# Lexmata/llama-gguf

Measured on AMD Instinct MI355X. Metric: decode tokens/sec Llama-3-8B Q4_K_M, 1 GPU; % of HBM roofline, higher is better.
Workload: dtype f32 (x as 4xint8 limbs on the matrix cores, exact int32 accumulation)

## Files before the change

### llama-gguf_amd/csrc/attention.hip

```cpp
#include <cstdlib>

#include "attn_split.h"
#include "tq_fwht.h"
#include "xq.h"
#include "prefill.h"
#include "timeline.h"

LGH_TL_DEFINE(attn)

namespace lgh {

template <int D, int G, int NW, bool PF = false, bool DIRECT = false, bool MULTI = false>
__global__ void __launch_bounds__(NW * 64) attn_partial_kernel(const float* __restrict__ q, const float* __restrict__ kc,
                                                           const float* __restrict__ vc, uint32_t max_seq, float scale,
                                                           const int* pos_ptr, int kv_len_fixed, uint32_t n_splits,
                                                           float* __restrict__ part_ml, float* __restrict__ part_acc,
                                                           const int* __restrict__ slot = nullptr, uint64_t slot_stride = 0) {
  constexpr int LPR = D / 4;
  constexpr int RPW = 64 / LPR;
  __shared__ float s_ml[NW * G * 2];
  __shared__ __attribute__((aligned(16))) float s_acc[NW * G * D];
  LGH_TL_BEGIN(attn, lgh::TL_ATTN, n_splits);

  const uint32_t kvh = blockIdx.x / n_splits, sp = blockIdx.x % n_splits;
// ... 43 lines not shown
#pragma unroll
    for (int j = 0; j < kAhead; j++)
      if (base + j * stride < kv_len) step(base + j * stride, kk[j], vv[j]);
  }

  attn_merge_rows<G, LPR>(m, l, acc);
  attn_stash<G, 4, LPR>(s_ml, s_acc, wave, sub, li, m, l, acc);
  __syncthreads();
  const size_t pbase = ((size_t)kvh * n_splits + sp) * G;
  for (uint32_t e = threadIdx.x; e < (uint32_t)(G * D); e += NW * 64) {
    const uint32_t g = e / D, dim = e % D;
    float mn, lsum, a;
    attn_merge_waves<NW, G, D>(s_ml, s_acc, g, dim, mn, lsum, a);
    if (DIRECT) {
      const float o = a * (1.0f / lsum);
      part_acc[(pbase + g) * D + dim] = o;
      if (part_ml) xq_store_chunk(reinterpret_cast<uint8_t*>(part_ml), (uint32_t)((pbase + g) * D + dim) >> 4, o);
    } else if (PF) {
      const _Float16 o = (_Float16)(a * (1.0f / lsum));
      *reinterpret_cast<_Float16*>(reinterpret_cast<uint8_t*>(part_acc) + xh_offset(blockIdx.y, (uint32_t)(pbase + g) * D + dim)) = o;
    } else {
      attn_store_partial<D>(part_ml, part_acc, pbase + g, dim, mn, lsum, a);
    }
  }
  LGH_TL_END();
}

__device__ __forceinline__ f32x4 unpack_i8x4(uint32_t w, float scale) {
  f32x4 r;
  r.x = (float)(int)(int8_t)(w & 0xFFu) * scale;
  r.y = (float)(int)(int8_t)((w >> 8) & 0xFFu) * scale;
  r.z = (float)(int)(int8_t)((w >> 16) & 0xFFu) * scale;
  r.w = (float)(int)(int8_t)(w >> 24) * scale;
  return r;
}

__device__ __forceinline__ float i8_row_scale(float amax) { return amax > 1e-10f ? amax / 127.0f : 1.0f; }
__device__ __forceinline__ uint32_t i8_quantize(float v, float scale) {
  float r = roundf(v / scale);
  r = r < -128.0f ? -128.0f : (r > 127.0f ? 127.0f : r);
  return (uint32_t)(int)r & 0xFFu;
}

template <int LPR>
__device__ __forceinline__ uint32_t quantize_row_i8(f32x4 x, float& scale) {
  float amax = fmaxf(fmaxf(fabsf(x.x), fabsf(x.y)), fmaxf(fabsf(x.z), fabsf(x.w)));
// ... 262 lines not shown
    constexpr int D = decltype(d)::value, G = decltype(gg)::value;
    return long_ctx ? attn_go<D, G, 8>(a) : attn_go<D, G, 4>(a);
  });
}

hipError_t attn_launch(const float* q, const float* kcache, const float* vcache, uint32_t n_heads, uint32_t n_kv,
                       uint32_t head_dim, uint32_t max_seq, float scale, const int* pos, int kv_len_fixed,
                       uint32_t n_splits, float* part_ml, float* part_acc, hipStream_t st) {
  if (n_kv == 0 || n_heads % n_kv) return hipErrorInvalidValue;
  return attn_split_dispatch(head_dim, n_heads / n_kv,
                             AttnArgs{q, kcache, vcache, n_kv, max_seq, scale, pos, kv_len_fixed, n_splits, part_ml, part_acc, st, 0, nullptr, 0});
}

hipError_t attn_direct_launch(const float* q, const float* kcache, const float* vcache, uint32_t n_heads, uint32_t n_kv, uint32_t head_dim,
                              uint32_t max_seq, float scale, const int* pos, float* out, uint8_t* xq_out, hipStream_t st) {
  if (n_kv == 0 || n_heads % n_kv || !pos) return hipErrorInvalidValue;
  return attn_dispatch(head_dim, n_heads / n_kv, [&](auto d, auto gg) {
    hipLaunchKernelGGL((attn_partial_kernel<decltype(d)::value, decltype(gg)::value, 16, false, true>), dim3(n_kv), dim3(1024), 0, st, q, kcache, vcache,
                       max_seq, scale, pos, 0, 1u, reinterpret_cast<float*>(xq_out), out);
    return hipGetLastError();
  });
}

struct PfTqEpi { const float* signs; float inv_scale, inv_d; };

template <int D, int NW, bool TQ>
__global__ void __launch_bounds__(NW * 64) attn_pf_mfma_kernel(const float* __restrict__ q, const float* __restrict__ kc, const float* __restrict__ vc,
                                                               uint32_t n_heads, uint32_t g_per_kv, uint32_t max_seq, float scale, uint32_t pos0,
                                                               uint32_t m_tokens, uint8_t* __restrict__ xh_out, const PfTqEpi tq) {
  constexpr int DJ = D / 4;
  constexpr int DQ = D / 16;
  constexpr int DP = D + 4;
  extern __shared__ __attribute__((aligned(16))) float pf_lds[];
  float (*s_o)[16][DP] = reinterpret_cast<float (*)[16][DP]>(pf_lds);
  float (*s_m)[16] = reinterpret_cast<float (*)[16]>(pf_lds + NW * 16 * DP);
  float (*s_l)[16] = s_m + NW;
  const uint32_t head = blockIdx.x, tt = blockIdx.y, kvh = head / g_per_kv;
  const uint32_t lane = threadIdx.x & 63, wave = threadIdx.x >> 6, n = lane & 15, c = lane >> 4;
  const uint32_t tok = tt * 16 + n, tokc = tok < m_tokens ? tok : m_tokens - 1;
  const uint32_t kv_last = pos0 + m_tokens - 1;
  const uint32_t n_tiles = (pos0 + tt * 16 + 16 + 15) / 16;
  float qf[DJ];
  {
    const float* qp = q + ((size_t)tokc * n_heads + head) * D + c * DJ;
#pragma unroll
    for (int j = 0; j < DJ; j += 4) {
// ... 249 lines not shown
```

### llama-gguf_amd/csrc/common.h

```cpp
#pragma once

#include <hip/hip_runtime.h>
#include <stdint.h>
#include <stddef.h>
#include <vector>

#include "../../include/llama_gguf_hip.h"

namespace lgh {

typedef uint32_t u32x4 __attribute__((ext_vector_type(4)));
typedef uint32_t u32x2 __attribute__((ext_vector_type(2)));
typedef float f32x4 __attribute__((ext_vector_type(4)));

constexpr int kWave = 64;
constexpr int kNumCU = 256;

__host__ __device__ inline uint32_t blk_elems(int t) {
  switch (t) {
    case LGH_TYPE_F32: case LGH_TYPE_F16: case LGH_TYPE_BF16: return 1;
    case LGH_TYPE_Q4_0: case LGH_TYPE_Q4_1: case LGH_TYPE_Q5_0: case LGH_TYPE_Q5_1: case LGH_TYPE_Q8_0:
    case LGH_TYPE_Q8_1: return 32;
    case LGH_TYPE_Q2_K: case LGH_TYPE_Q3_K: case LGH_TYPE_Q4_K: case LGH_TYPE_Q5_K: case LGH_TYPE_Q6_K:
    case LGH_TYPE_Q8_K: return 256;
// ... 159 lines not shown
                             uint32_t n_splits, float* part_ml, float* part_acc, hipStream_t st);
hipError_t attn_combine_multi_launch(const float* part_ml, const float* part_acc, uint32_t n_heads, uint32_t n_kv, uint32_t head_dim,
                                     uint32_t n_splits, uint32_t n_seq, float* out, uint8_t* xq_out, hipStream_t st);
hipError_t ewise_launch(int op, const float* a, const float* b, float s, float* out, uint64_t n, hipStream_t st);
hipError_t softmax_rows_launch(const float* x, float* out, uint32_t rows, uint32_t last_dim, hipStream_t st);
hipError_t matmul_f32_launch(const float* a, const float* b, float* c, uint32_t m, uint32_t k, uint32_t n, hipStream_t st);
hipError_t silu_mul_launch(const float* gate, const float* up, float* out, uint32_t n, hipStream_t st);
hipError_t argmax_launch(const float* logits, uint32_t n, float* part_val, int* part_idx, int* state, int* out_token,
                         hipStream_t st);
hipError_t argmax_merge_launch(const float* part_val, const int* part_idx, uint32_t nparts, int* state, int* out_token, hipStream_t st);
hipError_t advance_launch(int* state, hipStream_t st);
hipError_t copy_words_launch(void* dst, const void* src, uint32_t n_words, hipStream_t st);
hipError_t moe_group_launch(const int* sel, uint32_t n_seq, uint32_t top_k, uint32_t n_experts, int* cnt, int* idx, uint32_t idx_stride, hipStream_t st);
hipError_t moe_combine_launch(const float* tmp, const float* moe_w, uint32_t top_k, float* hidden, uint32_t H, uint32_t n_seq, const float* nw,
                              uint8_t* xq, uint32_t xq_stride, float* ssq, uint32_t ssq_stride, hipStream_t st);
hipError_t moe_router_launch(const float* x, const float* norm_w, float eps, const float* w, uint32_t hidden,
                             uint32_t n_experts, uint32_t top_k, int* sel, float* sel_w, hipStream_t st, uint32_t n_tokens = 1);

hipError_t attn_launch(const float* q, const float* kcache, const float* vcache, uint32_t n_heads, uint32_t n_kv,
                       uint32_t head_dim, uint32_t max_seq, float scale, const int* pos, int kv_len_fixed,
                       uint32_t n_splits, float* part_ml, float* part_acc, hipStream_t st);
hipError_t attn_direct_launch(const float* q, const float* kcache, const float* vcache, uint32_t n_heads, uint32_t n_kv, uint32_t head_dim,
                              uint32_t max_seq, float scale, const int* pos, float* out, uint8_t* xq_out, hipStream_t st);
bool attn_shape_has_fast_kernel(uint32_t head_dim, uint32_t group);
hipError_t kv_roundtrip_launch(int fmt, const float* x, uint32_t n, uint8_t* bytes, float* scale_out, float* back, hipStream_t st);
hipError_t attn_q8_launch(int fmt, const float* q, int8_t* k8, int8_t* v8, float* kscale, float* vscale, const float* k_new, const float* v_new,
                          uint32_t n_heads, uint32_t n_kv, uint32_t head_dim, uint32_t max_seq, float scale, const int* pos, uint32_t n_splits,
                          float* part_ml, float* part_acc, hipStream_t st);
hipError_t attn_q8_multi_launch(int fmt, const float* q, int8_t* k8, int8_t* v8, float* kscale, float* vscale, const float* k_new, const float* v_new,
                                uint32_t x_stride, uint32_t n_heads, uint32_t n_kv, uint32_t head_dim, uint32_t max_seq, float scale, const int* pos,
                                const int* slot, uint32_t n_seq, uint32_t n_splits, float* part_ml, float* part_acc, hipStream_t st);
hipError_t attn_tq_launch(int bits, const float* q, uint8_t* kq, uint8_t* vq, const float* k_new, const float* v_new, const float* signs,
                          uint32_t n_heads, uint32_t n_kv, uint32_t head_dim, uint32_t max_seq, float scale, const int* pos, uint32_t n_splits,
                          float* part_ml, float* part_acc, hipStream_t st, const float* qjl_s = nullptr, uint32_t* kx = nullptr);
hipError_t attn_tq_combine_launch(int bits, const float* part_ml, const float* part_acc, const float* signs, uint32_t n_heads, uint32_t n_kv,
                                  uint32_t head_dim, uint32_t n_splits, float* out, uint8_t* xq_out, hipStream_t st, uint32_t n_seq = 0,
                                  uint32_t xq_stride = 0);
hipError_t attn_tq_multi_launch(int bits, const float* q, uint8_t* kq, uint8_t* vq, const float* k_new, const float* v_new, const float* signs,
                                uint32_t n_heads, uint32_t n_kv, uint32_t head_dim, uint32_t max_seq, float scale, const int* pos, const int* slot,
                                uint64_t code_stride, uint64_t x_stride, uint32_t kv_stride, uint32_t n_seq, uint32_t n_splits, float* part_ml,
                                float* part_acc, hipStream_t st, const float* qjl_s = nullptr, uint32_t* kx = nullptr);
hipError_t tq_compress_launch(int bits, const float* x, uint32_t dim, const float* signs, uint8_t* out, hipStream_t st, const float* qjl_s = nullptr,
                              uint32_t* qjl_out = nullptr);
uint32_t tq_row_bytes_host(int bits, uint32_t d);
hipError_t tq_pf_rows_launch(int bits, float* kscr, float* vscr, uint8_t* kq, uint8_t* vq, float* q, const float* signs, uint32_t n_heads,
                             uint32_t n_kv, uint32_t head_dim, uint32_t max_seq, uint32_t pos0, uint32_t m_store, uint32_t m_q, uint32_t n_expand,
// ... 25 lines not shown
```

### llama-gguf_amd/csrc/device_utils.h

```cpp
#pragma once

#include "common.h"

namespace lgh {

__device__ __forceinline__ u32x4 ldg_nt128(const void* p) {
  return __builtin_nontemporal_load(reinterpret_cast<const u32x4*>(p));
}
__device__ __forceinline__ u32x2 ldg_nt64(const void* p) {
  return __builtin_nontemporal_load(reinterpret_cast<const u32x2*>(p));
}
__device__ __forceinline__ uint32_t ldg_nt32(const void* p) {
  return __builtin_nontemporal_load(reinterpret_cast<const uint32_t*>(p));
}
__device__ __forceinline__ uint16_t ldg_nt16(const void* p) {
  return __builtin_nontemporal_load(reinterpret_cast<const uint16_t*>(p));
}

__device__ __forceinline__ float h2f(uint32_t bits16) {
  _Float16 h;
  uint16_t b = (uint16_t)bits16;
  __builtin_memcpy(&h, &b, 2);
  return (float)h;
}
// ... 34 lines not shown
}

__device__ __forceinline__ float wave_sum(float v) {
#pragma unroll
  for (int off = 32; off >= 1; off >>= 1) v += __shfl_xor(v, off, 64);
  return v;
}

template <int CTRL, int ROW_MASK = 0xF>
__device__ __forceinline__ float dpp_f(float v) {
  return __builtin_bit_cast(float, __builtin_amdgcn_update_dpp(0, __builtin_bit_cast(int, v), CTRL, ROW_MASK, 0xF, false));
}

__device__ __forceinline__ float wave_sum_to_lane63(float v) {
  v += dpp_f<0xB1>(v);
  v += dpp_f<0x4E>(v);
  v += dpp_f<0x141>(v);
  v += dpp_f<0x140>(v);
  v += dpp_f<0x142, 0xA>(v);
  v += dpp_f<0x143, 0xC>(v);
  return v;
}

__device__ __forceinline__ float wave_max(float v) {
#pragma unroll
  for (int off = 32; off >= 1; off >>= 1) v = fmaxf(v, __shfl_xor(v, off, 64));
  return v;
}

__device__ __forceinline__ void amax_merge(float& bv, int& bi, float v, int i) {
  if (v > bv || (v == bv && i > bi)) { bv = v; bi = i; }
}

__device__ __forceinline__ void amax_block_reduce(float& bv, int& bi, float* sv, int* si) {
#pragma unroll
  for (int off = 32; off >= 1; off >>= 1) {
    float ov = __shfl_xor(bv, off, 64);
    int oi = __shfl_xor(bi, off, 64);
    amax_merge(bv, bi, ov, oi);
  }
  const uint32_t tid = threadIdx.x;
  if ((tid & 63) == 0) { sv[tid >> 6] = bv; si[tid >> 6] = bi; }
  __syncthreads();
  if (tid == 0) {
    for (uint32_t w = 1; w < (blockDim.x >> 6); w++) amax_merge(bv, bi, sv[w], si[w]);
  }
// ... 4 lines not shown
```

### llama-gguf_amd/csrc/engine.h

```cpp
#pragma once

#include <functional>
#include <string>
#include <vector>

#include "common.h"
#include "kv_cache.h"
#include "sample.h"

namespace lgh {

struct LayerW {
  bool owned = false;
  DevWeight wq, wk, wv, wo, gate, up, down;
  DevWeight gate_exps, up_exps, down_exps;
  float* attn_norm = nullptr;
  float* ffn_norm = nullptr;
  float* router = nullptr;
  float* bq = nullptr; float* bk = nullptr; float* bv = nullptr; float* bo = nullptr;
  KvCache kv;
  bool moe() const { return router != nullptr; }
};

enum TokenMode { MODE_PREFILL = 0, MODE_FORWARD = 1, MODE_GREEDY = 2, MODE_SAMPLE = 3, MODE_COUNT = 4 };

struct XqBuf { const float* f32 = nullptr; uint8_t* xq = nullptr; float* ssq = nullptr; uint32_t k = 0; bool fresh = false; const float* tag = nullptr; };

struct PfScratch {
  bool ready = false;
  uint8_t *xh_h = nullptr, *xh_attn = nullptr, *xh_act = nullptr;
  float *hidden = nullptr, *q = nullptr, *part = nullptr, *ssq = nullptr;
  size_t part_bytes = 0;
  int* tokens = nullptr;
  uint32_t* tok_pinned = nullptr;
  hipEvent_t tok_copied = nullptr;
  uint32_t tok_lo = 0, tok_hi = 0;
  int *moe_sel = nullptr, *moe_cnt = nullptr, *moe_base = nullptr, *moe_list = nullptr, *moe_rowmap = nullptr, *moe_tokmap = nullptr;
  float* moe_w = nullptr;
  uint8_t *xh_gather = nullptr, *xh_act_e = nullptr;
  float* tq_kv = nullptr;
};

struct ProfRec { int cls; int sym; uint64_t bytes; hipEvent_t a, b; };

struct BatchScratch {
  bool ready = false;
// ... 22 lines not shown
  lgh::KvLayout kvl;
  int device = 0;
  uint32_t l0 = 0, l1 = 0;
  bool first = true, last = true;
  hipStream_t own_stream = nullptr, stream = nullptr;
  std::vector<lgh::LayerW> layers;
  uint8_t* embd_raw = nullptr;
  int embd_type = -1;
  size_t embd_bytes = 0;
  std::vector<uint8_t> embd_host;
  lgh::DevWeight output;
  float* output_norm = nullptr;
  void *fwd_hidden = nullptr, *fwd_token = nullptr;
  float *hidden = nullptr, *xnorm = nullptr, *q = nullptr, *kv_tmp = nullptr, *attn_out = nullptr, *act = nullptr,
        *act2 = nullptr, *logits = nullptr, *part_ml = nullptr, *part_acc = nullptr, *rope_cs = nullptr, *moe_w = nullptr,
        *amax_v = nullptr;
  int *moe_sel = nullptr, *state = nullptr, *amax_i = nullptr, *tok_log = nullptr;
  uint32_t n_splits = 8;
  size_t pos = 0;
  bool finalized = false;
  bool profiling = false;
  std::string err;
  hipGraphExec_t graph[lgh::MODE_COUNT][2] = {};
  bool attn_direct = false;
  bool attn_generic = false;
  uint32_t direct_attn_max_kv = 0;
  uint64_t graph_nodes = 0;
  lgh_stats stats{};
  std::vector<lgh::ProfRec> prof;
  std::vector<void*> allocs;
  std::vector<lgh::XqBuf> xqs;
  lgh::PfScratch pf;
  lgh::BatchScratch batch;
  float* tq_signs = nullptr;
  std::vector<float> tq_signs_host;
  float* tq_qjl = nullptr;
  std::vector<float> tq_qjl_host;
  float* kv_shift_tmp = nullptr;
  lgh::SampBufs samp;
  lgh_sampler_config_ex samp_cfg{};
  bool samp_set = false;
};

#include <cstring>

int fail(lgh_ctx* c, int status, const std::string& msg);
#define HIP_TRY(c, status, expr)                                                                      \
// ... 138 lines not shown
```

### llama-gguf_amd/csrc/engine.hip

```cpp
#include "engine.h"
#include "prefill.h"
#include "xq.h"

#include <algorithm>
#include <cmath>
#include <cstdlib>
#include <cstring>

using namespace lgh;

constexpr uint32_t kDirectAttnDefaultKv = 64;

static int warm_kernels(lgh_ctx* c) {
  if (c->d.flags & LGH_FLAG_NO_GRAPH) return LGH_OK;
  int rc = LGH_OK;
  const bool keep_direct = c->attn_direct;
  for (int v = 0; v < 2 && !rc; v++) {
    if (v == 1 && c->direct_attn_max_kv == 0) continue;
    c->attn_direct = v == 1;
    HIP_TRY(c, LGH_OPERATION_FAILED, hipMemsetAsync(c->state, 0, ST_WORDS * 4, c->stream));
    for (int mode : {c->last ? MODE_GREEDY : MODE_PREFILL, MODE_PREFILL})
      if (!rc) rc = enqueue_token(c, mode);
  }
  c->attn_direct = keep_direct;
  for (auto& q : c->xqs) q.fresh = false;
  if (rc) return rc;
  if (c->samp.ctl && (rc = samp_warm(c, c->samp, c->logits, 1))) return rc;
  HIP_TRY(c, LGH_OPERATION_FAILED, hipMemsetAsync(c->state, 0, ST_WORDS * 4, c->stream));
  HIP_TRY(c, LGH_OPERATION_FAILED, hipStreamSynchronize(c->stream));
  return LGH_OK;
}

static int ensure_graph(lgh_ctx* c, int mode) {
  const int var = c->attn_direct ? 1 : 0;
  if (c->graph[mode][var]) return LGH_OK;
  size_t n_nodes = 0;
  const int rc = capture_graph(c, &c->graph[mode][var], [&] { return enqueue_token(c, mode); }, &n_nodes);
  if (n_nodes && (mode == MODE_GREEDY || (c->graph_nodes == 0 && mode != MODE_SAMPLE))) c->graph_nodes = n_nodes;
  return rc;
}

static int step(lgh_ctx* c, int mode) {
  if (c->pos >= c->d.max_seq_len)
    return fail(c, LGH_INVALID_ARGUMENT, "position " + std::to_string(c->pos) + " >= max_seq_len " + std::to_string(c->d.max_seq_len));
  int rc;
  c->attn_direct = c->pos + 1 <= c->direct_attn_max_kv;
  if (c->profiling || (c->d.flags & LGH_FLAG_NO_GRAPH)) {
    if ((rc = enqueue_token(c, mode))) return rc;
    if (c->profiling && (rc = drain_prof(c))) return rc;
  } else {
    if ((rc = ensure_graph(c, mode))) return rc;
    HIP_TRY(c, LGH_OPERATION_FAILED, hipGraphLaunch(c->graph[mode][c->attn_direct ? 1 : 0], c->stream));
  }
  c->pos += 1;
  c->stats.tokens_processed += 1;
  return LGH_OK;
}

static void drop_graphs(lgh_ctx* c) {
  for (int m = 0; m < MODE_COUNT; m++)
    for (int v = 0; v < 2; v++)
      if (c->graph[m][v]) { (void)hipGraphExecDestroy(c->graph[m][v]); c->graph[m][v] = nullptr; }
  for (auto& gg : c->batch.graph)
    for (auto& ge : gg)
      if (ge) { (void)hipGraphExecDestroy(ge); ge = nullptr; }
}

static int bind(const lgh_ctx* c) { return hipSetDevice(c->device) == hipSuccess ? LGH_OK : LGH_NOT_AVAILABLE; }

// ... 725 lines not shown
```

### llama-gguf_amd/csrc/engine_layer.hip

```cpp
#include "engine.h"
#include "xq.h"

#include <algorithm>
#include <cmath>

using namespace lgh;

namespace lgh {
hipError_t kv_store_launch(const float* k, const float* v, float* kcache, float* vcache, uint32_t n_kv, uint32_t d,
                           uint32_t max_seq, const int* pos, hipStream_t st);
}

void rope_table_host(const lgh_model_desc& d, std::vector<float>& cs) {
  const uint32_t half = d.head_dim / 2;
  cs.assign((size_t)d.max_seq_len * half * 2, 0.0f);
  for (uint32_t p = 0; p < d.max_seq_len; p++) {
    const float position = (float)p / d.rope_freq_scale;
    for (uint32_t i = 0; i < half; i++) {
      const float freq = 1.0f / std::pow(d.rope_freq_base, (float)(2 * i) / (float)d.head_dim);
      const float theta = position * freq;
      cs[((size_t)p * half + i) * 2] = std::cos(theta);
      cs[((size_t)p * half + i) * 2 + 1] = std::sin(theta);
    }
  }
// ... 130 lines not shown
    const float* signs = c->tq_signs + (size_t)(li - c->l0) * d.num_kv_heads * 2 * d.head_dim;
    const bool qjl = kvl.qjl();
    const float* qjl_s = qjl ? c->tq_qjl + (size_t)(li - c->l0) * d.num_kv_heads * d.head_dim * d.head_dim : nullptr;
    if ((rc = run_k(c, LGH_K_ATTN, LGH_SYM_ATTN, kv_bytes, [&] {
           return attn_tq_launch(bits, v.q, kv.k_bytes(), kv.v_bytes(), k_new, v_new, signs, d.num_heads, d.num_kv_heads, d.head_dim, d.max_seq_len,
                                 scale, pos, c->n_splits, c->part_ml, c->part_acc, c->stream, qjl_s, qjl ? kv.kx() : nullptr);
         })))
      return rc;
    uint8_t* const img = image();
    rc = run_k(c, LGH_K_ATTN_COMBINE, LGH_SYM_ATTN_COMBINE, 0, [&] {
      return attn_tq_combine_launch(bits, c->part_ml, c->part_acc, signs, d.num_heads, d.num_kv_heads, d.head_dim, c->n_splits, v.attn_out, img, c->stream);
    });
  } else if (kvl.staged()) {
    if ((rc = run_k(c, LGH_K_ATTN, LGH_SYM_ATTN, kv_bytes, [&] {
           return attn_q8_launch((int)d.kv_cache_type, v.q, kv.k_i8(), kv.v_i8(), kv.kscale(), kv.vscale(), k_new, v_new, d.num_heads, d.num_kv_heads, d.head_dim,
                                 d.max_seq_len, scale, pos, c->n_splits, c->part_ml, c->part_acc, c->stream);
         })))
      return rc;
    rc = merge(image());
  } else if (c->attn_generic) {
    rc = run_k(c, LGH_K_ATTN, LGH_SYM_ATTN, kv_bytes, [&] {
      return attn_decode_any_launch(v.q, kv.k_f32(), kv.v_f32(), v.attn_out, d.num_heads, d.num_kv_heads, d.head_dim, d.max_seq_len, scale, pos, c->stream);
    });
  } else if (c->attn_direct) {
    uint8_t* const img = image();
    rc = run_k(c, LGH_K_ATTN, LGH_SYM_ATTN, kv_bytes, [&] {
      return attn_direct_launch(v.q, kv.k_f32(), kv.v_f32(), d.num_heads, d.num_kv_heads, d.head_dim, d.max_seq_len, scale, pos, v.attn_out, img, c->stream);
    });
  } else {
    if ((rc = run_k(c, LGH_K_ATTN, LGH_SYM_ATTN, kv_bytes, [&] {
           return attn_launch(v.q, kv.k_f32(), kv.v_f32(), d.num_heads, d.num_kv_heads, d.head_dim, d.max_seq_len, scale, pos, 0, c->n_splits, c->part_ml,
                              c->part_acc, c->stream);
         })))
      return rc;
    rc = merge(image());
  }
  if (rc) return rc;
  if (qa) { qa->fresh = true; qa->tag = nullptr; }
  else xq_stale(c, v.attn_out);
  return LGH_OK;
}

static int layer_forward(lgh_ctx* c, uint32_t li, const float* next_nw, bool next_mfma) {
  LayerW& Lw = c->layers[li];
  const AttnView av{c->hidden, c->q, c->kv_tmp, c->attn_out};
  int rc;
  if ((rc = qkv_forward(c, Lw, av))) return rc;
// ... 75 lines not shown
```

### llama-gguf_amd/csrc/ops_api.hip

```cpp
#include "engine.h"
#include "xq.h"
#include "prefill.h"

#include <cmath>
#include <vector>

using namespace lgh;

#include <algorithm>

#ifdef LGH_STAMPS
namespace lgh { hipError_t pf_read_stamps(unsigned long long* host, size_t n); }
extern "C" int lgh_debug_pf_stamps(unsigned long long* out, size_t n) { return lgh::pf_read_stamps(out, n) == hipSuccess ? 0 : 10; }
namespace lgh { hipError_t mv_read_stamps(unsigned long long* host, size_t n); hipError_t mvq_read_stamps(unsigned long long* host, size_t n); hipError_t mvq_read_wave_stamps(unsigned long long* host, size_t n); hipError_t mvq_spans(unsigned long long* host, int reset); }
#include <cstdio>
#include "timeline.h"
namespace lgh { hipError_t tl_read_mvq(void*); hipError_t tl_read_attn(void*); hipError_t tl_read_deq(void*); hipError_t tl_read_misc(void*); }
extern "C" long long lgh_debug_timeline(int which, void* out) {
  if (!out) return (long long)sizeof(lgh::TlBuf);
  hipError_t e = which == 0 ? lgh::tl_read_mvq(out) : which == 1 ? lgh::tl_read_attn(out) : which == 2 ? lgh::tl_read_deq(out) : lgh::tl_read_misc(out);
  return e == hipSuccess ? 0 : -1;
}
#endif

// ... 513 lines not shown
float half_to_float(uint16_t h) {
  const uint32_t s = (uint32_t)(h >> 15) << 31, e = (h >> 10) & 0x1Fu, m = h & 0x3FFu;
  float v;
  if (e == 0) v = (float)m * 0x1p-24f;
  else if (e == 31) v = m ? NAN : INFINITY;
  else v = std::ldexp((float)(m | 0x400u), (int)e - 25);
  uint32_t b;
  std::memcpy(&b, &v, 4);
  b |= s;
  std::memcpy(&v, &b, 4);
  return v;
}

}

extern "C" {

int lgh_op_attention_decode(int device, int path, const float* q, const float* k_cache, const float* v_cache, float* out, size_t n_heads,
                            size_t n_kv, size_t head_dim, size_t max_seq, float scale, size_t pos, int n_splits, uint8_t* image_out) {
  Tmp t(device);
  if (t.rc) return t.rc;
  if (!q || !k_cache || !v_cache || !out || n_kv == 0 || n_heads % n_kv || head_dim == 0 || pos >= max_seq || max_seq > 0x7FFFFFFFu)
    return LGH_INVALID_ARGUMENT;
  if (path < 0 || path > 2 || (path == 2 && image_out)) return LGH_INVALID_ARGUMENT;
  const size_t g = n_heads / n_kv;
  const bool fast = attn_shape_has_fast_kernel((uint32_t)head_dim, (uint32_t)g);
  if (path != 2 && !fast) return LGH_UNSUPPORTED;
  if (path == 0 && (n_splits < 1 || n_splits > 32)) return LGH_INVALID_ARGUMENT;
  if (path == 2 && max_seq * 4 > 150 * 1024) return LGH_UNSUPPORTED;
  const AttnView v{nullptr, t.up(q, n_heads * head_dim), nullptr, t.up(nullptr, n_heads * head_dim)};
  if (!v.q || !v.attn_out) return LGH_ALLOCATION_FAILED;
  int rc;
  if ((rc = attn_setup(t, LGH_KV_F32, n_heads, n_kv, head_dim, max_seq, path == 0 ? n_splits : 0)) || (rc = set_pos(t, pos))) return rc;
  t.c->attn_direct = path == 1;
  t.c->attn_generic = path == 2;
  const void* const caches[KV_KINDS] = {k_cache, v_cache};
  return attn_run(t, v, caches, nullptr, scale, out, image_out);
}

int lgh_op_attention_decode_multi(int device, const float* q, const float* k_cache, const float* v_cache, float* out, size_t n_heads, size_t n_kv,
                                  size_t head_dim, size_t max_seq, size_t n_slots, size_t n_seq, const int* pos, const int* slot, float scale,
                                  int n_splits, uint8_t* image_out) {
  Tmp t(device);
  if (t.rc) return t.rc;
  if (!q || !k_cache || !v_cache || !out || !pos || !slot || n_kv == 0 || n_heads % n_kv || head_dim == 0 || max_seq == 0 || max_seq > 0x7FFFFFFFu ||
      n_slots == 0 || n_splits < 1 || n_splits > 32 || !seqs_ok(n_seq, kMaxBatch, slot, n_slots, false, pos, max_seq))
    return LGH_INVALID_ARGUMENT;
  if (!attn_shape_has_fast_kernel((uint32_t)head_dim, (uint32_t)(n_heads / n_kv))) return LGH_UNSUPPORTED;
  if (int rc = attn_multi_setup(t, LGH_KV_F32, q, nullptr, nullptr, n_heads, n_kv, head_dim, max_seq, n_seq, pos, slot, n_splits)) return rc;
  const void* const caches[KV_KINDS] = {k_cache, v_cache};
  return attn_multi_run(t, n_slots, n_seq, caches, nullptr, scale, out, image_out);
}

int lgh_op_attention_kv8(int device, uint32_t kv_cache_type, const float* q, int8_t* k_bytes, int8_t* v_bytes, float* k_scale, float* v_scale,
                         const float* k_new, const float* v_new, float* out, size_t n_heads, size_t n_kv, size_t head_dim, size_t max_seq,
                         float scale, size_t pos, int n_splits, uint8_t* image_out) {
  Tmp t(device);
// ... 1187 lines not shown
```

### llama-gguf_amd/csrc/tensor_parallel.hip

```cpp
#include "engine.h"
#include "xq.h"

#include <algorithm>
#include <cmath>
#include <cstring>

using namespace lgh;

namespace lgh {

constexpr int kTpMaxRanks = 8;
struct TpPeers { const float* p[kTpMaxRanks - 1]; };

template <int N>
__global__ void __launch_bounds__(64) tp_reduce_kernel(const float* p0, const float* resid, const float* nw, float* out, uint8_t* xq,
                                                       float* ssq, uint32_t H, TpPeers peers) {
  __shared__ __attribute__((aligned(16))) float s_v[320], s_h[320];
  const uint32_t lane = threadIdx.x, e0 = blockIdx.x * 256 + lane * 4;
  const bool ok = e0 < H;
  const uint32_t ec = ok ? e0 : 0;
  f32x4 p[N];
  p[0] = *reinterpret_cast<const f32x4*>(p0 + ec);
#pragma unroll
  for (int r = 1; r < N; r++) p[r] = *reinterpret_cast<const f32x4*>(peers.p[r - 1] + ec);
// ... 340 lines not shown
    for (size_t r = 1; r < n; r++) {
      TP_HIP(t, hipSetDevice(t->device[r]));
      if (stream_of(t->rank[r]) != c0->stream) TP_HIP(t, hipStreamWaitEvent(stream_of(t->rank[r]), t->token_back, 0));
    }
  }
#undef RANK_TRY
  return LGH_OK;
}

void tp_drop_graphs(lgh_tp* t) {
  for (auto& gm : t->graph)
    for (auto& ge : gm)
      if (ge) { (void)hipGraphExecDestroy(ge); ge = nullptr; }
}

bool tp_eager(const lgh_tp* t) { return !t->one_stream || (t->d.flags & LGH_FLAG_NO_GRAPH); }

int tp_step(lgh_tp* t, int mode) {
  if (t->pos >= t->d.max_seq_len)
    return tfail(t, LGH_INVALID_ARGUMENT, "position " + std::to_string(t->pos) + " >= max_seq_len " + std::to_string(t->d.max_seq_len));
  bool direct = false;
  for (lgh_ctx* c : t->rank) {
    c->pos = t->pos;
    c->attn_direct = c->pos + 1 <= c->direct_attn_max_kv;
    direct = c->attn_direct;
  }
  int rc;
  TP_HIP(t, hipSetDevice(t->device[0]));
  if (tp_eager(t)) {
    if ((rc = tp_enqueue(t, mode))) return rc;
  } else {
    lgh_ctx* c0 = t->rank[0];
    hipGraphExec_t& g = t->graph[mode][direct ? 1 : 0];
    if (!g) {
      size_t nodes = 0;
      int inner = LGH_OK;
      rc = capture_graph(c0, &g, [&] { return inner = tp_enqueue(t, mode); }, &nodes);
      if (rc) return inner ? rc : rank_fail(t, 0, rc);
      if (nodes && (mode == MODE_GREEDY || !t->graph_nodes)) t->graph_nodes = nodes;
    }
    TP_HIP(t, hipGraphLaunch(g, c0->stream));
  }
  t->pos += 1;
  for (lgh_ctx* c : t->rank) { c->pos = t->pos; c->stats.tokens_processed += 1; }
  return LGH_OK;
}

int tp_set_token(lgh_tp* t, uint32_t token) {
// ... 81 lines not shown
  for (size_t r = 0; r < n; r++) {
    lgh_ctx* c = t->rank[r];
    TP_HIP(t, hipSetDevice(t->device[r]));
    const AllocSpec bufs[] = {{(void**)&t->part[0][r], (size_t)H * 4}, {(void**)&t->part[1][r], (size_t)H * 4}};
    if ((rc = alloc_zeroed(c, bufs, 2, c->stats.scratch_bytes))) return rank_fail(t, r, rc);
    if (!t->one_stream)
      for (int w = 0; w < 3; w++) {
        t->ev[w].resize(n, nullptr);
        TP_HIP(t, hipEventCreateWithFlags(&t->ev[w][r], hipEventDisableTiming));
      }
  }
  if (!t->one_stream) {
    TP_HIP(t, hipSetDevice(t->device[0]));
    TP_HIP(t, hipEventCreateWithFlags(&t->token_back, hipEventDisableTiming));
  }
  t->finalized = true;
  t->pos = 0;
  if (!tp_eager(t)) {
    for (int v = 0; v < 2; v++) {
      if (v == 1 && t->rank[0]->direct_attn_max_kv == 0) continue;
      for (int mode : {MODE_GREEDY, MODE_PREFILL}) {
        for (lgh_ctx* c : t->rank) {
          c->pos = 0;
          c->attn_direct = v == 1;
          TP_HIP(t, hipMemsetAsync(c->state, 0, ST_WORDS * 4, c->stream));
        }
        if ((rc = tp_enqueue(t, mode))) return rc;
      }
    }
  }
  for (lgh_ctx* c : t->rank) {
    TP_HIP(t, hipSetDevice(c->device));
    c->pos = 0;
    for (auto& q : c->xqs) q.fresh = false;
    TP_HIP(t, hipMemsetAsync(c->state, 0, ST_WORDS * 4, c->stream));
  }
  return tp_sync_all(t);
}

void lgh_tp_destroy(lgh_tp* t) {
  if (!t) return;
  for (lgh_ctx* c : t->rank) (void)lgh_synchronize(c);
  tp_drop_graphs(t);
  for (auto& evs : t->ev)
    for (hipEvent_t e : evs)
      if (e) (void)hipEventDestroy(e);
  if (t->token_back) (void)hipEventDestroy(t->token_back);
// ... 123 lines not shown
```

### llama-gguf_amd/hip_backend.py

```python
from __future__ import annotations

import ctypes as C
import os
from typing import Iterable, Optional, Sequence

import numpy as np

_HERE = os.path.dirname(os.path.abspath(__file__))
LIB_PATH = os.path.join(_HERE, "lib", "libllama_gguf_hip%s.so" % ("_" + os.environ["LGH_LIB_VARIANT"] if os.environ.get("LGH_LIB_VARIANT") else ""))

ABI_SYMBOLS = (
    "lgh_device_count", "lgh_create", "lgh_upload_tensor", "lgh_finalize", "lgh_destroy", "lgh_forward",
    "lgh_prefill_token", "lgh_prefill_batch", "lgh_prefill_is_batched", "lgh_op_mat_mat",
    "lgh_op_kv_roundtrip", "lgh_op_add", "lgh_op_mul", "lgh_op_scale", "lgh_op_silu", "lgh_op_gelu", "lgh_op_softmax", "lgh_op_matmul", "lgh_op_matvec",
    "lgh_op_matvec_q", "lgh_op_attention", "lgh_backend_create", "lgh_backend_destroy", "lgh_backend_load_weight",
    "lgh_backend_has_weight", "lgh_backend_vec_mat_q", "lgh_backend_last_error", "lgh_reset", "lgh_position", "lgh_kv_truncate", "lgh_kv_shift_left", "lgh_stage_prefill_batch", "lgh_stage_hidden_block_buffer", "lgh_forward_argmax", "lgh_decode_greedy",
    "lgh_last_error", "lgh_get_stats", "lgh_set_profiling", "lgh_set_stream", "lgh_get_stream", "lgh_synchronize",
    "lgh_read_hidden", "lgh_stage_hidden_buffer", "lgh_stage_forward", "lgh_op_dequantize", "lgh_op_vec_mat",
    "lgh_op_rms_norm", "lgh_op_rope", "lgh_op_attention_cached", "lgh_op_silu_mul", "lgh_op_norm_vec_mat",
    "lgh_op_swiglu_vec_mat", "lgh_bench_vec_mat", "lgh_bench_hbm_read", "lgh_gguf_inspect", "lgh_load_gguf",
    "lgh_stage_io_buffers", "lgh_stage_set_forward_targets", "lgh_stage_step", "lgh_stage_read_tokens", "lgh_gguf_get", "lgh_stage_read_logits",
    "lgh_pipeline_create", "lgh_pipeline_upload_tensor", "lgh_pipeline_finalize", "lgh_pipeline_destroy", "lgh_pipeline_forward",
    "lgh_pipeline_prefill_token", "lgh_pipeline_decode_greedy", "lgh_pipeline_reset", "lgh_pipeline_position", "lgh_pipeline_kv_truncate", "lgh_pipeline_stages",
    "lgh_pipeline_last_error",
# ... 746 lines not shown
def op_rms_norm(x, w, eps: float, device: int = 0) -> np.ndarray:
    x, w = _f32(x), _f32(w)
    out = np.empty_like(x)
    _chk(load_library().lgh_op_rms_norm(device, x.ctypes.data, w.ctypes.data, eps, out.ctypes.data, x.size), "rms_norm")
    return out


def op_rope(q, k, pos: int, freq_base: float, freq_scale: float, neox: bool, device: int = 0):
    q, k = _f32(q).copy(), _f32(k).copy()
    _chk(load_library().lgh_op_rope(device, q.ctypes.data, k.ctypes.data, q.shape[0], k.shape[0], q.shape[1], pos,
                                    freq_base, freq_scale, int(neox)), "rope")
    return q, k


def op_attention_cached(q, k_cache, v_cache, scale: float, kv_len: int, n_splits: int = 8, device: int = 0) -> np.ndarray:
    q, kc, vc = _f32(q), _f32(k_cache), _f32(v_cache)
    out = np.empty_like(q)
    _chk(load_library().lgh_op_attention_cached(device, q.ctypes.data, kc.ctypes.data, vc.ctypes.data, out.ctypes.data,
                                                q.shape[0], kc.shape[0], q.shape[1], kc.shape[1], scale, kv_len,
                                                n_splits), "attention_cached")
    return out


ATTN_SPLIT, ATTN_DIRECT, ATTN_ANY = 0, 1, 2


def _attn_image(q, n_images: int = 1):
    nb = _xq_bytes(q.shape[-2] * q.shape[-1])
    return np.zeros(nb if n_images == 1 else (n_images, nb), np.uint8)


def op_attention_decode(path: int, q, k_cache, v_cache, scale: float, pos: int, n_splits: int = 8, device: int = 0, *, image: bool = False):
    q, kc, vc = _f32(q), _f32(k_cache), _f32(v_cache)
    out = np.empty_like(q)
    img = _attn_image(q) if image else None
    _chk(load_library().lgh_op_attention_decode(device, path, q.ctypes.data, kc.ctypes.data, vc.ctypes.data, out.ctypes.data, q.shape[0],
                                                kc.shape[0], q.shape[1], kc.shape[1], scale, pos, n_splits, _ptr(img)), "attention_decode")
    return (out, img) if image else out


def op_attention_decode_multi(q, k_cache, v_cache, scale: float, pos, slot, n_splits: int = 8, device: int = 0, *, image: bool = False):
    q, kc, vc = _f32(q), _f32(k_cache), _f32(v_cache)
    pos, slot = np.ascontiguousarray(pos, dtype=np.int32), np.ascontiguousarray(slot, dtype=np.int32)
    out = np.empty_like(q)
    img = _attn_image(q, q.shape[0] + 1) if image else None
    _chk(load_library().lgh_op_attention_decode_multi(device, q.ctypes.data, kc.ctypes.data, vc.ctypes.data, out.ctypes.data, q.shape[1],
                                                      kc.shape[1], q.shape[2], kc.shape[2], kc.shape[0], q.shape[0], pos.ctypes.data,
# ... 678 lines not shown
```

Baseline: 689.5.

## Add per-head single-launch decode attention kernel and widen direct-path KV threshold

Adds a new decode attention kernel that runs one 1024-thread block per query head (grid n_kv x G). It stores all scores in LDS, computes softmax in two passes and accumulates V with a four-deep register ring of K/V prefetches, so no split-merge pass is needed. Short contexts now use this kernel instead of the grouped direct kernel, and the KV length that selects the single-launch path rises from 64 to 256. The aim is more blocks in flight, which better fills the GPU and hides latency for short sequences. The cost is that K/V are re-read once per query head in a group rather than once per KV head, and LDS use grows with the row cap.

```diff
diff --git a/llama-gguf_amd/csrc/attention.hip b/llama-gguf_amd/csrc/attention.hip
--- a/llama-gguf_amd/csrc/attention.hip
+++ b/llama-gguf_amd/csrc/attention.hip
@@ -89,6 +89,154 @@
     } else {
       attn_store_partial<D>(part_ml, part_acc, pbase + g, dim, mn, lsum, a);
     }
+  }
+  LGH_TL_END();
+}
+
+template <int D, int G>
+__global__ void __launch_bounds__(1024) attn_head_kernel(const float* __restrict__ q, const float* __restrict__ kc, const float* __restrict__ vc,
+                                                         const int* pos_ptr, float* __restrict__ out, uint8_t* __restrict__ xq_out, uint32_t max_seq,
+                                                         float scale, uint32_t cap_rows) {
+  constexpr int NW = 16, CH = 128;
+  constexpr int NB = D / 32;
+  constexpr int LPR = D / 4, RPW = 64 / LPR;
+  static_assert(NW * RPW * NB == CH && NW * 8 == CH, "a chunk is one K sweep and NB V sweeps");
+  extern __shared__ __attribute__((aligned(16))) float ah_lds[];
+  float* const s_sc = ah_lds;
+  float* const s_p = s_sc + cap_rows;
+  float* const s_acc = s_p + cap_rows;
+  float* const s_sum = s_acc + NW * D;
+  LGH_TL_BEGIN(attn, lgh::TL_ATTN, 1);
+
+  const uint32_t kvh = blockIdx.x, head = kvh * G + blockIdx.y;
+  const uint32_t lane = threadIdx.x & 63, wave = __builtin_amdgcn_readfirstlane(threadIdx.x >> 6);
+  const uint32_t kl = lane & 7, ksub = lane >> 3;
+  const uint32_t li = lane % LPR, vsub = lane / LPR;
+  f32x4 qv[NB];
+#pragma unroll
+  for (int j = 0; j < NB; j++) qv[j] = *reinterpret_cast<const f32x4*>(q + (size_t)head * D + j * 32 + kl * 4);
+  uint32_t kv_len = sload_u32(pos_ptr) + 1;
+  kv_len = kv_len < cap_rows ? kv_len : cap_rows;
+  const uint32_t n_ch = (kv_len + CH - 1) / CH, last = kv_len - 1;
+
+  const char* const kbase = reinterpret_cast<const char*>(kc + (size_t)kvh * max_seq * D);
+  const char* const vbase = reinterpret_cast<const char*>(vc + (size_t)kvh * max_seq * D);
+  const uint32_t krow0 = wave * 8 + ksub, vrow0 = wave * RPW + vsub;
+  auto k_has = [&](uint32_t c) { return c * CH + wave * 8 < kv_len; };
+  auto load_k = [&](f32x4 (&k)[NB], uint32_t c) {
+    const uint32_t r = c * CH + krow0, off = (r < last ? r : last) * (D * 4) + kl * 16;
+#pragma unroll
+    for (int j = 0; j < NB; j++) k[j] = __builtin_nontemporal_load(reinterpret_cast<const f32x4*>(kbase + off + j * 128));
+  };
+  auto load_v = [&](f32x4 (&v)[NB], uint32_t c) {
+#pragma unroll
+    for (int j = 0; j < NB; j++) {
+      const uint32_t r = c * CH + j * (NW * RPW) + vrow0, off = (r < last ? r : last) * (D * 4) + li * 16;
+      v[j] = __builtin_nontemporal_load(reinterpret_cast<const f32x4*>(vbase + off));
+    }
+  };
+  const bool longc = n_ch > 2;
+  auto load_k_or_v = [&](f32x4 (&b)[NB], uint32_t kch, uint32_t vch) {
+    const char* const base = longc ? kbase : vbase;
+    const uint32_t rk = kch * CH + krow0, offk = (rk < last ? rk : last) * (D * 4) + kl * 16;
+#pragma unroll
+    for (int j = 0; j < NB; j++) {
+      const uint32_t rv = vch * CH + j * (NW * RPW) + vrow0, offv = (rv < last ? rv : last) * (D * 4) + li * 16;
+      b[j] = __builtin_nontemporal_load(reinterpret_cast<const f32x4*>(base + (longc ? offk + j * 128 : offv)));
+    }
+  };
+  f32x4 buf[4][NB];
+  load_k(buf[0], 0);
+  load_k(buf[1], 1);
+#pragma unroll
+  for (int j = 0; j < NB; j++) qv[j] = qv[j] * scale;
+
+  auto score = [&](const f32x4 (&k)[NB], uint32_t c) {
+    if (!k_has(c)) return;
+    float s = qv[0].x * k[0].x;
+    s = __builtin_fmaf(qv[0].y, k[0].y, s); s = __builtin_fmaf(qv[0].z, k[0].z, s); s = __builtin_fmaf(qv[0].w, k[0].w, s);
+#pragma unroll
+    for (int j = 1; j < NB; j++) {
+      s = __builtin_fmaf(qv[j].x, k[j].x, s); s = __builtin_fmaf(qv[j].y, k[j].y, s);
+      s = __builtin_fmaf(qv[j].z, k[j].z, s); s = __builtin_fmaf(qv[j].w, k[j].w, s);
+    }
+    s += dpp_f<0xB1>(s);
+    s += dpp_f<0x4E>(s);
+    s += dpp_f<0x141>(s);
+    const uint32_t r = c * CH + krow0;
+    if (kl == 0 && r < kv_len) s_sc[r] = s;
+  };
+  load_k_or_v(buf[2], 2, 0);
+  load_k_or_v(buf[3], 3, 1);
+  uint32_t c = 0;
+  for (; c + 4 < n_ch; c += 4) {
+#pragma unroll
+    for (int i = 0; i < 4; i++) { score(buf[i], c + i); load_k(buf[i], c + 4 + i); }
+  }
+  score(buf[0], c);
+  score(buf[1], c + 1);
+  if (longc) {
+    score(buf[2], c + 2);
+    load_v(buf[2], 0);
+    score(buf[3], c + 3);
+    load_v(buf[3], 1);
+    load_v(buf[0], 2);
+    load_v(buf[1], 3);
+  }
+  __syncthreads();
+
+  float mx = kNegBig;
+  for (uint32_t b = 0; b < kv_len; b += 64) {
+    const uint32_t r = b + lane;
+    const float s = s_sc[r < last ? r : last];
+    mx = s > mx ? s : mx;
+  }
+  mx = wave_max_dpp(mx);
+  float ps = 0.0f;
+  for (uint32_t b = wave * 64; b < n_ch * CH; b += NW * 64) {
+    const uint32_t r = b + lane;
+    const float p = r < kv_len ? __expf(s_sc[r < last ? r : last] - mx) : 0.0f;
+    s_p[r] = p;
+    ps += p;
+  }
+  ps = wave_sum_to_lane63(ps);
+  if (lane == 63) s_sum[wave] = ps;
+  __syncthreads();
+
+  f32x4 acc = (f32x4)(0.0f);
+  auto accum = [&](const f32x4 (&v)[NB], uint32_t c) {
+    if (c >= n_ch) return;
+    float p[NB];
+#pragma unroll
+    for (int j = 0; j < NB; j++) p[j] = s_p[c * CH + j * (NW * RPW) + vrow0];
+#pragma unroll
+    for (int j = 0; j < NB; j++) {
+      acc.x = __builtin_fmaf(p[j], v[j].x, acc.x); acc.y = __builtin_fmaf(p[j], v[j].y, acc.y);
+      acc.z = __builtin_fmaf(p[j], v[j].z, acc.z); acc.w = __builtin_fmaf(p[j], v[j].w, acc.w);
+    }
+  };
+  for (c = 0; c + 4 < n_ch; c += 4) {
+#pragma unroll
+    for (int i = 0; i < 4; i++) { accum(buf[(i + 2) & 3], c + i); load_v(buf[(i + 2) & 3], c + 4 + i); }
+  }
+#pragma unroll
+  for (int i = 0; i < 4; i++) accum(buf[(i + 2) & 3], c + i);
+
+#pragma unroll
+  for (int off = LPR; off < 64; off <<= 1) {
+    acc.x += __shfl_xor(acc.x, off, 64); acc.y += __shfl_xor(acc.y, off, 64);
+    acc.z += __shfl_xor(acc.z, off, 64); acc.w += __shfl_xor(acc.w, off, 64);
+  }
+  if (vsub == 0) *reinterpret_cast<f32x4*>(&s_acc[wave * D + li * 4]) = acc;
+  __syncthreads();
+  if (threadIdx.x < (uint32_t)D) {
+    const uint32_t dim = threadIdx.x;
+    float o = s_acc[dim], sum = s_sum[0];
+#pragma unroll
+    for (int w = 1; w < NW; w++) { o += s_acc[w * D + dim]; sum += s_sum[w]; }
+    o = o * (1.0f / sum);
+    out[(size_t)head * D + dim] = o;
+    if (xq_out) xq_store_chunk(xq_out, (head * D + dim) >> 4, o);
   }
   LGH_TL_END();
 }
@@ -397,6 +545,27 @@
   });
 }
 
+template <int D, int G>
+static hipError_t attn_head_go(const float* q, const float* kc, const float* vc, uint32_t n_kv, uint32_t max_seq, float scale, const int* pos,
+                               uint32_t cap_rows, float* out, uint8_t* xq_out, hipStream_t st) {
+  auto lds = [](uint32_t rows) { return (size_t)(2 * rows + 16 * D + 16) * 4; };
+  static bool attr_set[64] = {};
+  if (hipError_t e = lds_opt_in(reinterpret_cast<const void*>(&attn_head_kernel<D, G>), (int)lds(kAttnHeadMaxRows), attr_set); e != hipSuccess) return e;
+  hipLaunchKernelGGL((attn_head_kernel<D, G>), dim3(n_kv, G), dim3(1024), lds(cap_rows), st, q, kc, vc, pos, out, xq_out, max_seq, scale, cap_rows);
+  return hipGetLastError();
+}
+
+hipError_t attn_head_launch(const float* q, const float* kcache, const float* vcache, uint32_t n_heads, uint32_t n_kv, uint32_t head_dim,
+                            uint32_t max_seq, float scale, const int* pos, uint32_t max_rows, float* out, uint8_t* xq_out, hipStream_t st) {
+  if (n_kv == 0 || n_heads % n_kv || !pos || max_rows == 0 || max_seq == 0) return hipErrorInvalidValue;
+  const uint32_t rows = max_rows < max_seq ? max_rows : max_seq;
+  if (rows > kAttnHeadMaxRows) return hipErrorInvalidValue;
+  const uint32_t cap_rows = (rows + 127) / 128 * 128;
+  return attn_dispatch(head_dim, n_heads / n_kv, [&](auto d, auto gg) {
+    return attn_head_go<decltype(d)::value, decltype(gg)::value>(q, kcache, vcache, n_kv, max_seq, scale, pos, cap_rows, out, xq_out, st);
+  });
+}
+
 struct PfTqEpi { const float* signs; float inv_scale, inv_d; };
 
 template <int D, int NW, bool TQ>
diff --git a/llama-gguf_amd/csrc/common.h b/llama-gguf_amd/csrc/common.h
--- a/llama-gguf_amd/csrc/common.h
+++ b/llama-gguf_amd/csrc/common.h
@@ -205,6 +205,9 @@
                        uint32_t n_splits, float* part_ml, float* part_acc, hipStream_t st);
 hipError_t attn_direct_launch(const float* q, const float* kcache, const float* vcache, uint32_t n_heads, uint32_t n_kv, uint32_t head_dim,
                               uint32_t max_seq, float scale, const int* pos, float* out, uint8_t* xq_out, hipStream_t st);
+constexpr uint32_t kAttnHeadMaxRows = 16384;
+hipError_t attn_head_launch(const float* q, const float* kcache, const float* vcache, uint32_t n_heads, uint32_t n_kv, uint32_t head_dim,
+                            uint32_t max_seq, float scale, const int* pos, uint32_t max_rows, float* out, uint8_t* xq_out, hipStream_t st);
 bool attn_shape_has_fast_kernel(uint32_t head_dim, uint32_t group);
 hipError_t kv_roundtrip_launch(int fmt, const float* x, uint32_t n, uint8_t* bytes, float* scale_out, float* back, hipStream_t st);
 hipError_t attn_q8_launch(int fmt, const float* q, int8_t* k8, int8_t* v8, float* kscale, float* vscale, const float* k_new, const float* v_new,
diff --git a/llama-gguf_amd/csrc/device_utils.h b/llama-gguf_amd/csrc/device_utils.h
--- a/llama-gguf_amd/csrc/device_utils.h
+++ b/llama-gguf_amd/csrc/device_utils.h
@@ -80,6 +80,21 @@
   return v;
 }
 
+template <int CTRL, int ROW_MASK = 0xF>
+__device__ __forceinline__ float dpp_max(float v) {
+  const int b = __builtin_bit_cast(int, v);
+  return fmaxf(v, __builtin_bit_cast(float, __builtin_amdgcn_update_dpp(b, b, CTRL, ROW_MASK, 0xF, false)));
+}
+__device__ __forceinline__ float wave_max_dpp(float v) {
+  v = dpp_max<0xB1>(v);
+  v = dpp_max<0x4E>(v);
+  v = dpp_max<0x141>(v);
+  v = dpp_max<0x140>(v);
+  v = dpp_max<0x142, 0xA>(v);
+  v = dpp_max<0x143, 0xC>(v);
+  return __builtin_bit_cast(float, __builtin_amdgcn_readlane(__builtin_bit_cast(int, v), 63));
+}
+
 __device__ __forceinline__ float wave_max(float v) {
 #pragma unroll
   for (int off = 32; off >= 1; off >>= 1) v = fmaxf(v, __shfl_xor(v, off, 64));
diff --git a/llama-gguf_amd/csrc/engine.h b/llama-gguf_amd/csrc/engine.h
--- a/llama-gguf_amd/csrc/engine.h
+++ b/llama-gguf_amd/csrc/engine.h
@@ -22,6 +22,7 @@
   bool moe() const { return router != nullptr; }
 };
 
+enum AttnVariant : uint8_t { ATTN_VAR_SPLIT = 0, ATTN_VAR_DIRECT = 1, ATTN_VAR_HEAD = 2 };
 enum TokenMode { MODE_PREFILL = 0, MODE_FORWARD = 1, MODE_GREEDY = 2, MODE_SAMPLE = 3, MODE_COUNT = 4 };
 
 struct XqBuf { const float* f32 = nullptr; uint8_t* xq = nullptr; float* ssq = nullptr; uint32_t k = 0; bool fresh = false; const float* tag = nullptr; };
@@ -90,7 +91,7 @@
   bool profiling = false;
   std::string err;
   hipGraphExec_t graph[lgh::MODE_COUNT][2] = {};
-  bool attn_direct = false;
+  lgh::AttnVariant attn_direct = lgh::ATTN_VAR_SPLIT;
   bool attn_generic = false;
   uint32_t direct_attn_max_kv = 0;
   uint64_t graph_nodes = 0;
diff --git a/llama-gguf_amd/csrc/engine.hip b/llama-gguf_amd/csrc/engine.hip
--- a/llama-gguf_amd/csrc/engine.hip
+++ b/llama-gguf_amd/csrc/engine.hip
@@ -9,15 +9,15 @@
 
 using namespace lgh;
 
-constexpr uint32_t kDirectAttnDefaultKv = 64;
+constexpr uint32_t kDirectAttnDefaultKv = 256;
 
 static int warm_kernels(lgh_ctx* c) {
   if (c->d.flags & LGH_FLAG_NO_GRAPH) return LGH_OK;
   int rc = LGH_OK;
-  const bool keep_direct = c->attn_direct;
+  const AttnVariant keep_direct = c->attn_direct;
   for (int v = 0; v < 2 && !rc; v++) {
     if (v == 1 && c->direct_attn_max_kv == 0) continue;
-    c->attn_direct = v == 1;
+    c->attn_direct = v == 1 ? ATTN_VAR_HEAD : ATTN_VAR_SPLIT;
     HIP_TRY(c, LGH_OPERATION_FAILED, hipMemsetAsync(c->state, 0, ST_WORDS * 4, c->stream));
     for (int mode : {c->last ? MODE_GREEDY : MODE_PREFILL, MODE_PREFILL})
       if (!rc) rc = enqueue_token(c, mode);
@@ -44,7 +44,7 @@
   if (c->pos >= c->d.max_seq_len)
     return fail(c, LGH_INVALID_ARGUMENT, "position " + std::to_string(c->pos) + " >= max_seq_len " + std::to_string(c->d.max_seq_len));
   int rc;
-  c->attn_direct = c->pos + 1 <= c->direct_attn_max_kv;
+  c->attn_direct = c->pos + 1 <= c->direct_attn_max_kv ? ATTN_VAR_HEAD : ATTN_VAR_SPLIT;
   if (c->profiling || (c->d.flags & LGH_FLAG_NO_GRAPH)) {
     if ((rc = enqueue_token(c, mode))) return rc;
     if (c->profiling && (rc = drain_prof(c))) return rc;
diff --git a/llama-gguf_amd/csrc/engine_layer.hip b/llama-gguf_amd/csrc/engine_layer.hip
--- a/llama-gguf_amd/csrc/engine_layer.hip
+++ b/llama-gguf_amd/csrc/engine_layer.hip
@@ -176,7 +176,16 @@
     rc = run_k(c, LGH_K_ATTN, LGH_SYM_ATTN, kv_bytes, [&] {
       return attn_decode_any_launch(v.q, kv.k_f32(), kv.v_f32(), v.attn_out, d.num_heads, d.num_kv_heads, d.head_dim, d.max_seq_len, scale, pos, c->stream);
     });
-  } else if (c->attn_direct) {
+  } else if (c->attn_direct == ATTN_VAR_HEAD) {
+    if (c->pos + 1 > c->direct_attn_max_kv)
+      return fail(c, LGH_INVALID_ARGUMENT, "single-launch attention at position " + std::to_string(c->pos) + " past its " +
+                                               std::to_string(c->direct_attn_max_kv) + " rows");
+    uint8_t* const img = image();
+    rc = run_k(c, LGH_K_ATTN, LGH_SYM_ATTN, kv_bytes, [&] {
+      return attn_head_launch(v.q, kv.k_f32(), kv.v_f32(), d.num_heads, d.num_kv_heads, d.head_dim, d.max_seq_len, scale, pos, c->direct_attn_max_kv,
+                              v.attn_out, img, c->stream);
+    });
+  } else if (c->attn_direct == ATTN_VAR_DIRECT) {
     uint8_t* const img = image();
     rc = run_k(c, LGH_K_ATTN, LGH_SYM_ATTN, kv_bytes, [&] {
       return attn_direct_launch(v.q, kv.k_f32(), kv.v_f32(), d.num_heads, d.num_kv_heads, d.head_dim, d.max_seq_len, scale, pos, v.attn_out, img, c->stream);
diff --git a/llama-gguf_amd/csrc/ops_api.hip b/llama-gguf_amd/csrc/ops_api.hip
--- a/llama-gguf_amd/csrc/ops_api.hip
+++ b/llama-gguf_amd/csrc/ops_api.hip
@@ -559,17 +559,19 @@
   if (t.rc) return t.rc;
   if (!q || !k_cache || !v_cache || !out || n_kv == 0 || n_heads % n_kv || head_dim == 0 || pos >= max_seq || max_seq > 0x7FFFFFFFu)
     return LGH_INVALID_ARGUMENT;
-  if (path < 0 || path > 2 || (path == 2 && image_out)) return LGH_INVALID_ARGUMENT;
+  if (path < 0 || path > 3 || (path == 2 && image_out)) return LGH_INVALID_ARGUMENT;
   const size_t g = n_heads / n_kv;
   const bool fast = attn_shape_has_fast_kernel((uint32_t)head_dim, (uint32_t)g);
   if (path != 2 && !fast) return LGH_UNSUPPORTED;
   if (path == 0 && (n_splits < 1 || n_splits > 32)) return LGH_INVALID_ARGUMENT;
   if (path == 2 && max_seq * 4 > 150 * 1024) return LGH_UNSUPPORTED;
+  if (path == 3 && max_seq > kAttnHeadMaxRows) return LGH_UNSUPPORTED;
   const AttnView v{nullptr, t.up(q, n_heads * head_dim), nullptr, t.up(nullptr, n_heads * head_dim)};
   if (!v.q || !v.attn_out) return LGH_ALLOCATION_FAILED;
   int rc;
   if ((rc = attn_setup(t, LGH_KV_F32, n_heads, n_kv, head_dim, max_seq, path == 0 ? n_splits : 0)) || (rc = set_pos(t, pos))) return rc;
-  t.c->attn_direct = path == 1;
+  t.c->attn_direct = path == 1 ? ATTN_VAR_DIRECT : path == 3 ? ATTN_VAR_HEAD : ATTN_VAR_SPLIT;
+  if (path == 3) t.c->direct_attn_max_kv = (uint32_t)max_seq;
   t.c->attn_generic = path == 2;
   const void* const caches[KV_KINDS] = {k_cache, v_cache};
   return attn_run(t, v, caches, nullptr, scale, out, image_out);
diff --git a/llama-gguf_amd/csrc/tensor_parallel.hip b/llama-gguf_amd/csrc/tensor_parallel.hip
--- a/llama-gguf_amd/csrc/tensor_parallel.hip
+++ b/llama-gguf_amd/csrc/tensor_parallel.hip
@@ -386,8 +386,8 @@
   bool direct = false;
   for (lgh_ctx* c : t->rank) {
     c->pos = t->pos;
-    c->attn_direct = c->pos + 1 <= c->direct_attn_max_kv;
-    direct = c->attn_direct;
+    c->attn_direct = c->pos + 1 <= c->direct_attn_max_kv ? ATTN_VAR_HEAD : ATTN_VAR_SPLIT;
+    direct = c->attn_direct != ATTN_VAR_SPLIT;
   }
   int rc;
   TP_HIP(t, hipSetDevice(t->device[0]));
@@ -515,7 +515,7 @@
       for (int mode : {MODE_GREEDY, MODE_PREFILL}) {
         for (lgh_ctx* c : t->rank) {
           c->pos = 0;
-          c->attn_direct = v == 1;
+          c->attn_direct = v == 1 ? ATTN_VAR_HEAD : ATTN_VAR_SPLIT;
           TP_HIP(t, hipMemsetAsync(c->state, 0, ST_WORDS * 4, c->stream));
         }
         if ((rc = tp_enqueue(t, mode))) return rc;
diff --git a/llama-gguf_amd/hip_backend.py b/llama-gguf_amd/hip_backend.py
--- a/llama-gguf_amd/hip_backend.py
+++ b/llama-gguf_amd/hip_backend.py
@@ -792,7 +792,7 @@
     return out
 
 
-ATTN_SPLIT, ATTN_DIRECT, ATTN_ANY = 0, 1, 2
+ATTN_SPLIT, ATTN_DIRECT, ATTN_ANY, ATTN_HEAD = 0, 1, 2, 3
 
 
 def _attn_image(q, n_images: int = 1):
```

New measurement: 699.6 (median of 6 runs). 1.01x the previous value.
